# vsislab/Controllable_XGating

Measured on AMD Instinct MI355X. Metric: decoder timesteps/sec (train fwd+bwd) at batch 128, MSRVTT 26x1536+1024, higher is better.
Workload: dtype f32; 1 GPU; configs[1]: 1xMI355X batch 128 per GPU teacher-forced XE train, 26 frames x (1536+1024), hidden 512, att 1536, emb 468, vocab 20000, seq_len 20 (T=21), fp32; global_batch=128, per_gpu_batch=128, parallelism=dp1, gemm_precision=fp32, zero_grad=fused into the update, launch=eager kernel launches

## Files before the change

### controllable_xgating_amd/_native.py

```python
from __future__ import annotations

import ctypes as C
import os

_HERE = os.path.dirname(os.path.abspath(__file__))
LIB_PATH = os.environ.get("XG_LIBRARY") or os.path.join(_HERE, "lib", "libxgate_hip.so")
LIB_DIAG_PATH = os.path.join(_HERE, "lib", "libxgate_hip_diag.so")

XG_VERSION = 206
XG_ROLLOUT_GREEDY, XG_ROLLOUT_SAMPLE, XG_ROLLOUT_REPLAY = 0, 1, 2


class XgDims(C.Structure):
    _fields_ = [(n, C.c_int32) for n in ("B", "K", "R", "A", "E", "V", "C", "H", "F1", "F2", "T")]


class XgBnState(C.Structure):
    _fields_ = [(n, C.c_void_p) for n in ("rgb_mean", "rgb_var", "opfl_mean", "opfl_var")]


class XgBatch(C.Structure):
    _fields_ = [(n, C.c_void_p) for n in ("feats_rgb", "feats_opfl", "feat_mask", "pos_feats", "seq", "seq_mask")]


# ... 79 lines not shown
        "xg_nll_bwd": [vp, vp, vp, vp, i32, i32, i32, i32, vp, f32, vp, vp],
        "xg_clip_adam": [vp, i64, vp, vp, vp, vp, f32, f32, f32, f32, f32, i32, f32],
        "xg_clip_adam_zero": [vp, i64, vp, vp, vp, vp, f32, f32, f32, f32, f32, i32, f32],
        "xg_workspace_init": [vp, vp, C.c_size_t],
        "xg_adam_tick": [vp, vp, f32, f32],
        "xg_clip_adam_dev": [vp, i64, vp, vp, vp, vp, vp, f32, f32, f32, f32, f32, i32],
        "xg_pack_weights": [vp, PD, PP, vp, C.c_size_t, i32, i32],
        "xg_pack_weights_part": [vp, PD, PP, vp, C.c_size_t, i32, i32, i32],
        "xg_reward_fwd": [vp, vp, i32, vp, i32, vp, i32, i32, vp, i32, i32, vp],
        "xg_reward_bwd": [vp, vp, i32, vp, i32, i32, vp, i32, i32, vp, vp, vp, i32],
    }
    missing = [n for n in sigs if not hasattr(L, n)]
    if missing:
        raise XgError("%s (xg_version %d) lacks %s: rebuild it with `python __graft_entry__.py --force`"
                      % (LIB_PATH, L.xg_version(), ", ".join(missing)))
    for name, args in sigs.items():
        fn = getattr(L, name)
        fn.restype = C.c_int
        fn.argtypes = args
    L.xg_abi_check.restype = C.c_int
    L.xg_abi_check.argtypes = [C.c_int] + [C.c_size_t] * 5
    if L.xg_abi_check(XG_VERSION, C.sizeof(XgDims), C.sizeof(_XgParams), C.sizeof(XgBnState), C.sizeof(XgBatch), C.sizeof(XgRun)):
        raise XgError("%s has ABI version %d / other struct layouts than this binding (XG_VERSION %d): rebuild it with "
                      "`python __graft_entry__.py --force`" % (LIB_PATH, L.xg_version(), XG_VERSION))
    _lib = L
    return L


def check(rc: int, what: str):
    if rc != 0:
# ... 14 lines not shown
```

### controllable_xgating_amd/csrc/xg_gemm.hip

```cpp
#include "xg_common.h"
#include "xg_kernels.h"
#include <cstdio>
#include <cstdlib>
#include <type_traits>

typedef float f32x16 __attribute__((ext_vector_type(16)));
typedef float f32x4 __attribute__((ext_vector_type(4)));

namespace {

constexpr int BKS = 32;
constexpr int LDK = BKS + 4;
constexpr int MCP = 4;

template <int ROWS, bool KC>
struct TileGeom {
    static constexpr int lds_floats = KC ? ROWS * LDK : BKS * (ROWS + MCP);
    static constexpr int nvec = ROWS * BKS / 4 / 256;
};

template <int ROWS, bool KC, bool VEC>
__device__ __forceinline__ void load_tile(const float* __restrict__ P, int ld, int r0, int k0, int nrows, int K,
                                          f32x4 (&regs)[TileGeom<ROWS, KC>::nvec]) {
    constexpr int NV = TileGeom<ROWS, KC>::nvec;
// ... 124 lines not shown
                    acc[i][j] = __builtin_amdgcn_mfma_f32_32x32x2f32(fa[i][kk], fb[j][kk], acc[i][j], 0, 0, 0);
    }
}

struct GemmArgs {
    const float* A; const float* B; float* C; const float* bias;
    int M, N, K, lda, ldb, ldc, relu, accumulate;
    int splitk;
    int fast;
    int gm;
    int bg;
    float* csum[3];
    int alone;
};

template <int BM>
__device__ __forceinline__ void csum_flush(const f32x4& cs, f32x4* red4, int m0, int M, float* const (&out)[3]) {
    constexpr int RG = BM / 4;
    const int t = threadIdx.x;
    if (t < RG) {
        f32x4 v = cs;
#pragma unroll
        for (int j = 1; j < 256 / RG; ++j) v += red4[t + j * RG];
#pragma unroll
        for (int q = 0; q < 4; ++q) {
            const int row = m0 + 4 * t + q;
            if (row < M) {
#pragma unroll
                for (int o = 0; o < 3; ++o) if (out[o]) unsafeAtomicAdd(out[o] + row, v[q]);
            }
        }
    }
}

template <int BM, int BN, bool AKC, bool BKC, bool VEC>
__global__ void __launch_bounds__(256) gemm_kernel(GemmArgs g) {
    constexpr int WM = BM / 2, WN = BN / 2;
    constexpr int MT = WM / 32, NT = WN / 32;
    constexpr int A_FL = TileGeom<BM, AKC>::lds_floats;
    constexpr int B_FL = TileGeom<BN, BKC>::lds_floats;
    extern __shared__ __attribute__((aligned(16))) float smem[];
    constexpr int STAGE = A_FL + B_FL;

    const int ntm = (g.M + BM - 1) / BM, ntn = (g.N + BN - 1) / BN;
    const int nwg = ntm * ntn * g.splitk;
    int bid = blockIdx.x;
    {
        const int q = nwg / 8, r = nwg % 8, xcd = bid % 8, idx = bid / 8;
        bid = (xcd < r ? xcd * (q + 1) : r * (q + 1) + (xcd - r) * q) + idx;
    }
    const int ks = bid % g.splitk;
    bid /= g.splitk;
    int tm, tn;
    {
        const int per = g.gm * ntn, grp = bid / per, in = bid - grp * per;
        const int first = grp * g.gm, gsz = min(ntm - first, g.gm);
        tn = in / gsz;
        tm = first + (in - tn * gsz);
    }
    const int m0 = tm * BM, n0 = tn * BN;

    const int lane = threadIdx.x & 63, wave = threadIdx.x >> 6;
    const int wm = wave >> 1, wn = wave & 1;
    const int half = lane >> 5, l31 = lane & 31;

    f32x16 acc[MT][NT];
#pragma unroll
    for (int i = 0; i < MT; ++i)
#pragma unroll
        for (int j = 0; j < NT; ++j)
#pragma unroll
            for (int r = 0; r < 16; ++r) acc[i][j][r] = 0.f;

// ... 1 lines not shown
    f32x4 ra[NVA], rb[NVB];
    const int nslab_all = (g.K + BKS - 1) / BKS;
    const int s_begin = (int)(((long)ks * nslab_all) / g.splitk), s_end = (int)(((long)(ks + 1) * nslab_all) / g.splitk);
    const int nslab = s_end;
    uint32_t offA[NVA], offB[NVB];
    const bool fast = VEC && g.fast;
    if (fast) {
        tile_offsets<BM, AKC>(g.lda, m0, g.M, offA);
        tile_offsets<BN, BKC>(g.ldb, n0, g.N, offB);
    }
    const size_t stepA = (AKC ? (size_t)BKS : (size_t)BKS * g.lda) * sizeof(float);
    const size_t stepB = (BKC ? (size_t)BKS : (size_t)BKS * g.ldb) * sizeof(float);
    const int nfull = g.K / BKS;
    load_tile<BM, AKC, VEC>(g.A, g.lda, m0, s_begin * BKS, g.M, g.K, ra);
    load_tile<BN, BKC, VEC>(g.B, g.ldb, n0, s_begin * BKS, g.N, g.K, rb);
    const bool do_cs = !AKC && VEC && g.csum[0] != nullptr && tn == 0;
    f32x4 cs = {0.f, 0.f, 0.f, 0.f};
    if (do_cs) {
#pragma unroll
        for (int i = 0; i < NVA; ++i) cs += ra[i];
    }
    store_tile<BM, AKC>(smem, ra);
    store_tile<BN, BKC>(smem + A_FL, rb);
    __syncthreads();

    for (int s = s_begin; s < nslab; ++s) {
        const int cur = (s - s_begin) & 1;
        if (s + 1 < nslab) {
            if (fast && s + 1 < nfull) {
                load_fast<NVA>(reinterpret_cast<const char*>(g.A) + (size_t)(s + 1) * stepA, offA, ra);
                load_fast<NVB>(reinterpret_cast<const char*>(g.B) + (size_t)(s + 1) * stepB, offB, rb);
// ... 30 lines not shown
            if (col >= g.N) continue;
            const float bv = (g.bias && ks == 0) ? g.bias[col] : 0.f;
#pragma unroll
            for (int r = 0; r < 16; ++r) {
                const int row = m0 + wm * WM + i * 32 + (r & 3) + 8 * (r >> 2) + 4 * half;
                if (row < g.M) {
                    float* dst = g.C + (size_t)row * g.ldc + col;
                    float v = acc[i][j][r] + bv;
                    if (g.splitk > 1) { unsafeAtomicAdd(dst, v); continue; }
                    if (g.accumulate) v += *dst;
                    if (g.relu) v = fmaxf(v, 0.f);
                    *dst = v;
                }
            }
        }
}

template <int ROWS, int BK, bool KC>
struct TileW {
    static constexpr int ld = KC ? BK + 4 : ROWS + MCP;
    static constexpr int lds_floats = KC ? ROWS * (BK + 4) : BK * (ROWS + MCP);
    static constexpr int nvec = ROWS * BK / 4 / 256;
    static_assert(ROWS * BK % 1024 == 0, "tile must divide over 256 threads");
};
template <int ROWS, int BK, bool KC>
__device__ __forceinline__ void w1_offsets(int ld, int r0, int nrows, uint32_t (&off)[TileW<ROWS, BK, KC>::nvec]) {
    const int t = threadIdx.x;
#pragma unroll
    for (int i = 0; i < TileW<ROWS, BK, KC>::nvec; ++i) {
        const int f = t + 256 * i;
// ... 523 lines not shown
        XG_TRY(xg_lds_optin(optin, reinterpret_cast<const void*>(&gemm_kernel<BM, BN, AKC, BKC, VEC>), (int)lds));
    }
    hipLaunchKernelGGL((gemm_kernel<BM, BN, AKC, BKC, VEC>), dim3(ntm * ntn * g.splitk), dim3(256), lds, st, g);
    XG_CHECK_LAUNCH();
    return XG_OK;
}

struct TdArgs {
    const float* A; const float* B; float* C;
    int M, N, K, lda, ldb, ldc, accumulate;
    int ntm, ntn, ksplit, nrounds;
    float* csum[3];
};
constexpr int TD_LDW = 68;

template <int D>
__global__ void __launch_bounds__(256) gemm_td_kernel(TdArgs g) {
    extern __shared__ __attribute__((aligned(16))) float smem[];
    const int lane = threadIdx.x & 63, wave = __builtin_amdgcn_readfirstlane(threadIdx.x >> 6);
    const int a16 = lane & 15, kq = lane >> 4;
    const int G = gridDim.x;
    const int xq = G >> 3, xr = G & 7, xcd = blockIdx.x & 7, idx = blockIdx.x >> 3;
    const int pos = (xcd < xr ? xcd * (xq + 1) : xr * (xq + 1) + (xcd - xr) * xq) + idx;
    const int nitems = g.ntm * g.ntn * g.ksplit;
    const bool want_cs = g.csum[0] != nullptr;
    const size_t stepA = (size_t)16 * g.lda * sizeof(float), stepB = (size_t)16 * g.ldb * sizeof(float);
    float* red = smem + 4 * 64 * TD_LDW;
    for (int item = pos; item < nitems; item += G) {
        const int part = item % g.ksplit, tile = item / g.ksplit;
        const int tn = tile % g.ntn, tm = tile / g.ntn;
        const int m0 = tm * 64, n0 = tn * 64;
        const int i0 = (int)(((long)part * g.nrounds) / g.ksplit), i1 = (int)(((long)(part + 1) * g.nrounds) / g.ksplit);
        const bool cs_on = want_cs && tn == 0;
        const uint32_t offA = (uint32_t)(((size_t)kq * g.lda + min(m0 + 4 * a16, g.M - 4)) * sizeof(float));
        const uint32_t offB = (uint32_t)(((size_t)kq * g.ldb + min(n0 + 4 * a16, g.N - 4)) * sizeof(float));
        const char* pa = reinterpret_cast<const char*>(g.A) + (size_t)4 * wave * g.lda * sizeof(float);
        const char* pb = reinterpret_cast<const char*>(g.B) + (size_t)4 * wave * g.ldb * sizeof(float);
        f32x4 acc[4][4];
#pragma unroll
        for (int i = 0; i < 4; ++i)
#pragma unroll
            for (int j = 0; j < 4; ++j) acc[i][j] = f32x4{0.f, 0.f, 0.f, 0.f};
        f32x4 cs = {0.f, 0.f, 0.f, 0.f};
        f32x4 ra[D], rb[D];
        const char* qa = pa + (size_t)i0 * stepA;
        const char* qb = pb + (size_t)i0 * stepB;
#pragma unroll
        for (int u = 0; u < D; ++u) {
            ra[u] = *reinterpret_cast<const f32x4*>(qa + u * stepA + offA);
            rb[u] = *reinterpret_cast<const f32x4*>(qb + u * stepB + offB);
        }
        qa += D * stepA; qb += D * stepB;
// ... 40 lines not shown
                v += __shfl_xor(v, 32);
                if (kq == 0) red[wave * 64 + 4 * a16 + q] = v;
            }
        }
        __syncthreads();
        {
            const bool atom = g.ksplit > 1;
#pragma unroll
            for (int u = 0; u < 4; ++u) {
                const int q = lane + 64 * u;
                const int row = 16 * wave + (q >> 4), col = (q & 15) << 2;
                f32x4 v = *reinterpret_cast<const f32x4*>(smem + row * TD_LDW + col);
#pragma unroll
                for (int w2 = 1; w2 < 4; ++w2) v += *reinterpret_cast<const f32x4*>(smem + (w2 * 64 + row) * TD_LDW + col);
                const int gr = m0 + row, gc = n0 + col;
                if (gr < g.M && gc < g.N) {
                    float* dst = g.C + (size_t)gr * g.ldc + gc;
                    if (atom) {
#pragma unroll
                        for (int e = 0; e < 4; ++e) unsafeAtomicAdd(dst + e, v[e]);
                    } else if (g.accumulate) {
                        *reinterpret_cast<f32x4*>(dst) = *reinterpret_cast<const f32x4*>(dst) + v;
                    } else {
                        *reinterpret_cast<f32x4*>(dst) = v;
                    }
                }
            }
            if (cs_on && threadIdx.x < 64) {
                const int m = m0 + (int)threadIdx.x;
                if (m < g.M) {
                    const float v = (red[threadIdx.x] + red[64 + threadIdx.x]) + (red[128 + threadIdx.x] + red[192 + threadIdx.x]);
#pragma unroll
                    for (int o = 0; o < 3; ++o) if (g.csum[o]) unsafeAtomicAdd(g.csum[o] + m, v);
                }
            }
        }
        __syncthreads();
    }
}

int launch_td(hipStream_t st, const GemmArgs& a) {
    static const int off = xg_diag_env("XG_GEMM_NO_TD") ? 1 : 0;
    if (off || !a.fast || a.relu || a.bias || a.M % 4 || a.N % 4 || a.K % 16 || a.ldc % 4 || ((uintptr_t)a.C % 16) != 0) return 1;
    if (a.M < 64 || a.N < 64 || a.K < 16 * 16) return 1;
    TdArgs g{a.A, a.B, a.C, a.M, a.N, a.K, a.lda, a.ldb, a.ldc, a.accumulate, 0, 0, 1, a.K / 16, {a.csum[0], a.csum[1], a.csum[2]}};
    g.ntm = xg_cdiv(a.M, 64); g.ntn = xg_cdiv(a.N, 64);
    const long tiles = (long)g.ntm * g.ntn;
    if (tiles < 32) return 1;
    static const int td_all = xg_diag_env("XG_TD_ALL") ? atoi(xg_diag_env("XG_TD_ALL")) : 0;
    if (!td_all && !a.bg && !a.alone && tiles < 1024) return 1;
    static const int ks_env = xg_diag_env("XG_TD_KS") ? atoi(xg_diag_env("XG_TD_KS")) : 0;
    int ks = 1;
    if (tiles < 192) { ks = (int)(256 / tiles); if (ks > g.nrounds / 16) ks = g.nrounds / 16; if (ks < 1) ks = 1; }
    if (ks_env > 0) ks = ks_env;
    if (ks > g.nrounds / 8) ks = g.nrounds / 8;
    g.ksplit = ks;
    if (ks > 1 && !a.accumulate) {
        if (a.ldc == a.N) { if (hipMemsetAsync(a.C, 0, sizeof(float) * (size_t)a.M * a.N, st) != hipSuccess) return XG_EHIP; }
        else if (hipMemset2DAsync(a.C, sizeof(float) * a.ldc, 0, sizeof(float) * a.N, a.M, st) != hipSuccess) return XG_EHIP;
    }
    static const int bg_off = xg_diag_env("XG_GEMM_NO_BG") ? 1 : 0;
    const bool bg = a.bg && !bg_off;
    const long items = tiles * ks;
    const int GMAX = bg ? 256 : 512;
    const long rounds = xg_cdiv64(items, GMAX);
    const int G = (int)xg_cdiv64(items, rounds);
    size_t lds = (4 * 64 * TD_LDW + 256) * sizeof(float);
    if (bg && lds < 82 * 1024) lds = 82 * 1024;
    static const int depth_all = xg_diag_env("XG_TD_DEPTH") ? atoi(xg_diag_env("XG_TD_DEPTH")) : 8;
    const int depth_env = depth_all;
    if (depth_env == 4) {
        static std::atomic<unsigned> optin4{0};
        XG_TRY(xg_lds_optin(optin4, reinterpret_cast<const void*>(&gemm_td_kernel<4>), 84 * 1024));
        hipLaunchKernelGGL((gemm_td_kernel<4>), dim3(G), dim3(256), lds, st, g);
    } else if (depth_env == 12 && g.nrounds / ks >= 12) {
        static std::atomic<unsigned> optin12{0};
        XG_TRY(xg_lds_optin(optin12, reinterpret_cast<const void*>(&gemm_td_kernel<12>), 84 * 1024));
        hipLaunchKernelGGL((gemm_td_kernel<12>), dim3(G), dim3(256), lds, st, g);
    } else {
        static std::atomic<unsigned> optin{0};
        XG_TRY(xg_lds_optin(optin, reinterpret_cast<const void*>(&gemm_td_kernel<8>), 84 * 1024));
        hipLaunchKernelGGL((gemm_td_kernel<8>), dim3(G), dim3(256), lds, st, g);
    }
    XG_CHECK_LAUNCH();
    return XG_OK;
}
// ... 81 lines not shown
        }
    }
    if (vec && !force) {
        const int rc1 = dispatch_w1<AKC, BKC>(st, g);
        if (rc1 != 1) return rc1;
    }
    if (vec && !force) {
        const int rc = launch_pk<128, 128, AKC, BKC>(st, g, 40);
        if (rc != 1) return rc;
    }
    g.gm = xgk_group_rows(g.K / g.splitk);
    if (big) return vec ? launch<128, 128, AKC, BKC, true>(st, g) : launch<128, 128, AKC, BKC, false>(st, g);
    return vec ? launch<64, 64, AKC, BKC, true>(st, g) : launch<64, 64, AKC, BKC, false>(st, g);
}

}

int xgk_gemm(hipStream_t st, int mode, bool transA, bool transB, int M, int N, int K, const float* A, int lda,
             const float* B, int ldb, float* C, int ldc, const float* bias, bool relu, bool accumulate) {
    return xgk_gemm_cs(st, mode, transA, transB, M, N, K, A, lda, B, ldb, C, ldc, bias, relu, accumulate, nullptr, nullptr, nullptr);
}

int xgk_gemm_cs(hipStream_t st, int mode, bool transA, bool transB, int M, int N, int K, const float* A, int lda,
                const float* B, int ldb, float* C, int ldc, const float* bias, bool relu, bool accumulate, float* cs1, float* cs2,
                float* cs3) {
    if (M <= 0 || N <= 0) return XG_OK;
    if (K < 0 || !A || !B || !C) return XG_EINVAL;
    const bool want_cs = cs1 != nullptr;
    if (want_cs && !transA) return XG_EINVAL;
    const int bg = (mode & XGK_GEMM_BG) ? 1 : 0, alone = (mode & XGK_GEMM_ALONE) ? 1 : 0;
// ... 31 lines not shown
        return xgk_gemm_bf16x(st, 1 | (mode & XGK_GEMM_BG), transA, transB, M, N, K, A, A16, lda, B, B16, ldb, C, ldc, bias, relu, accumulate, cs1, cs2, cs3);
    }
    return xgk_gemm_cs(st, mode, transA, transB, M, N, K, A, lda, B, ldb, C, ldc, bias, relu, accumulate, cs1, cs2, cs3);
}

extern "C" int xg_gemm_mode(void* stream, int mode, int transA, int transB, int M, int N, int K, const float* A, int lda,
                            const float* B, int ldb, float* C, int ldc, const float* bias, int relu, int accumulate) {
    if (mode != 0 && mode != 1 && mode != 3) return XG_EINVAL;
    if (mode == 0 || M <= 0 || N <= 0)
        return xgk_gemm((hipStream_t)stream, 0, transA != 0, transB != 0, M, N, K, A, lda, B, ldb, C, ldc, bias, relu != 0, accumulate != 0);
    if (K < 0 || !A || !B || !C) return XG_EINVAL;
    return xgk_gemm_bf16((hipStream_t)stream, mode, transA != 0, transB != 0, M, N, K, A, lda, B, ldb, C, ldc, bias,
                         relu != 0, accumulate != 0);
}

extern "C" int xg_gemm(void* stream, int transA, int transB, int M, int N, int K, const float* A, int lda,
                       const float* B, int ldb, float* C, int ldc, const float* bias, int relu, int accumulate) {
    return xgk_gemm((hipStream_t)stream, 0, transA != 0, transB != 0, M, N, K, A, lda, B, ldb, C, ldc, bias,
                    relu != 0, accumulate != 0);
}
```

### controllable_xgating_amd/csrc/xg_kernels.h

```cpp
#pragma once
#include "xg_common.h"
#include "xg_select.h"
#include "xg_beam_core.h"
#include <cstddef>

static inline int xgk_group_rows(int k_depth) {
    const int g = 4096 / (k_depth > 0 ? k_depth : 1);
    return g < 1 ? 1 : (g > 8 ? 8 : g);
}
enum { XGK_GEMM_BG = 0x100,
       XGK_GEMM_ALONE = 0x200 };
int xgk_gemm(hipStream_t st, int mode, bool transA, bool transB, int M, int N, int K, const float* A, int lda,
             const float* B, int ldb, float* C, int ldc, const float* bias, bool relu, bool accumulate);
int xgk_gemm_cs(hipStream_t st, int mode, bool transA, bool transB, int M, int N, int K, const float* A, int lda,
                const float* B, int ldb, float* C, int ldc, const float* bias, bool relu, bool accumulate, float* cs1, float* cs2,
                float* cs3);
int xgk_gemm_x(hipStream_t st, int mode, bool transA, bool transB, int M, int N, int K, const float* A, const unsigned short* A16,
               int lda, const float* B, const unsigned short* B16, int ldb, float* C, int ldc, const float* bias, bool relu,
               bool accumulate, float* cs1 = nullptr, float* cs2 = nullptr, float* cs3 = nullptr);
int xgk_gemm_bf16(hipStream_t st, int planes, bool transA, bool transB, int M, int N, int K, const float* A, int lda,
                  const float* B, int ldb, float* C, int ldc, const float* bias, bool relu, bool accumulate, float* cs1 = nullptr,
                  float* cs2 = nullptr, float* cs3 = nullptr);
int xgk_gemm_bf16x(hipStream_t st, int planes, bool transA, bool transB, int M, int N, int K, const float* A, const unsigned short* A16,
                   int lda, const float* B, const unsigned short* B16, int ldb, float* C, int ldc, const float* bias, bool relu,
                   bool accumulate, float* cs1 = nullptr, float* cs2 = nullptr, float* cs3 = nullptr);
bool xgk_gemm_g16_ok(bool transA, bool transB, int M, int N, int K, const unsigned short* A16, int lda, const unsigned short* B16, int ldb);
int xgk_gemm_g16(hipStream_t st, bool transA, bool transB, int M, int N, int K, const unsigned short* A16, int lda,
                 const unsigned short* B16, int ldb, float* C, int ldc, const float* bias, bool relu, bool accumulate, int splitk,
                 float* cs1, float* cs2, float* cs3);
int xgk_cvt_bf16(hipStream_t st, const float* src, unsigned short* dst, size_t n);
static inline int xgk_linear(hipStream_t st, int mode, int M, int N, int K, const float* X, int ldx, const float* W,
                             const float* bias, float* Y, int ldy, bool relu = false, bool acc = false) {
    return xgk_gemm(st, mode, false, true, M, N, K, X, ldx, W, K, Y, ldy, bias, relu, acc);
}
// ... 237 lines not shown
```

### controllable_xgating_amd/csrc/xg_model.hip

```cpp
#include "xg_common.h"
#include <cstring>
#include "xg_kernels.h"
#include "../../include/xgate_beam.h"
#include "../../include/xgate_control.h"
#include "../../include/xgate_beam_control.h"

#include <new>
#include <cstdlib>

namespace {

constexpr int XG_NEV = 64, XG_NRING = 56;
struct XgAux { uint32_t magic; int device; hipStream_t s = nullptr, s2 = nullptr; hipEvent_t ev[XG_NEV]; };
constexpr uint32_t XG_AUX_MAGIC = 0x58474158u;
XgAux* aux_of(const XgRun* run) {
    static const bool disabled = xg_diag_env("XG_NO_OVERLAP") != nullptr;
    if (disabled || !run || !run->aux) return nullptr;
    XgAux* a = static_cast<XgAux*>(run->aux);
    int dev = -1;
    if (a->magic != XG_AUX_MAGIC || hipGetDevice(&dev) != hipSuccess || dev != a->device) return nullptr;
    return a;
}

struct Streams {
// ... 144 lines not shown
    return (!event || hipEventRecord(static_cast<hipEvent_t>(event), st) == hipSuccess) ? XG_OK : XG_EHIP;
}

inline int gemm_nn(hipStream_t st, int mode, int M, int N, int Kc, const float* dY, int lddy, const float* W, int ldw,
                   float* dX, int lddx, bool acc) {
    return xgk_gemm(st, mode, false, false, M, N, Kc, dY, lddy, W, ldw, dX, lddx, nullptr, false, acc);
}
inline int gemm_tn(hipStream_t st, int mode, int Mrows, int N, int K, const float* dY, int lddy, const float* X, int ldx,
                   float* dW, int lddw) {
    return xgk_gemm(st, mode, true, false, N, K, Mrows, dY, lddy, X, ldx, dW, lddw, nullptr, false, true);
}

inline int gemm_tn_cs(hipStream_t st, int mode, int Mrows, int N, int K, const float* dY, int lddy, const float* X, int ldx,
                      float* dW, int lddw, float* b1, float* b2 = nullptr, float* b3 = nullptr) {
    return xgk_gemm_cs(st, mode, true, false, N, K, Mrows, dY, lddy, X, ldx, dW, lddw, nullptr, false, true, b1, b2, b3);
}

inline const unsigned short* m16(const Ws& w, const float* p) {
    return (w.gm == 1 && w.sh16 && p >= w.base_f && p < w.end_f) ? w.sh16 + (p - w.base_f) : nullptr;
}
inline int cvt16(hipStream_t st, const Ws& w, const float* p, size_t n) {
    if (w.gm != 1 || n == 0) return XG_OK;
    if (!w.sh16) return XG_OK;
    const unsigned short* dst = m16(w, p);
    if (!dst) return XG_EINVAL;
    return xgk_cvt_bf16(st, p, const_cast<unsigned short*>(dst), n);
}
inline const unsigned short* w16(const Ws& w, int which) {
    return (w.gm == 1 && w.packed && w.pk.dtype == 1) ? w.pk.w16[which] : nullptr;
}
// ... 225 lines not shown
                sk.job[m].seg[0] = seg_nn(w, mo[m].pkb, w.dS[m] + (size_t)i * 4 * R, K * 4 * R, mo[m].whh, R, 4 * R);
            }
            XG_TRY(xgk_skinny(st, sk, sk_mode(w)));
        }
    }
    for (int m = 0; m < 2; ++m) XG_TRY(cvt16(st, w, w.dS[m], (size_t)N * 4 * R));
    const int gm_tail = w.gm | XGK_GEMM_ALONE;
    XG_TRY(ss.fork2());
    for (int m = 0; m < 2; ++m) {
        const EncMod &e = mo[m], &ge = gr[m];
        if (m == 0) XG_TRY(ss.fork());
        ZERO(sx, w.Hprev[m], (size_t)N * R);
        if (K > 1)
            XG_TRY(xgk_copy2d(sx, w.Hprev[m] + R, K * R, w.Hs[m], K * R, B, (K - 1) * R, false));
        XG_TRY(cvt16(sx, w, w.Hprev[m], (size_t)N * R));
        XG_TRY(tn16(sx, gm_tail, N, 4 * R, R, w.dS[m], m16(w, w.dS[m]), 4 * R, w.Hprev[m], m16(w, w.Hprev[m]), R, ge.whh, R, ge.bih, ge.bhh));
        XG_TRY(tn16(sx, gm_tail, N, 4 * R, R, w.dS[m], m16(w, w.dS[m]), 4 * R, w.X[m], m16(w, w.X[m]), R, ge.wih, R));
        hipStream_t sm = (m == 1 && ss.overlap()) ? ss.aux2 : st;
        XG_TRY(nn16(sm, w.gm, N, R, 4 * R, w.dS[m], m16(w, w.dS[m]), 4 * R, e.wih, w16(w, e.w16_wih), R, w.dX[m], R, false));
        if (!w.zeroed) { ZERO(sm, w.bn_s1[m], R); ZERO(sm, w.bn_s2[m], R); }
        XG_TRY(xgk_bn_bwd_reduce(sm, w.dX[m], w.X[m], w.Z[m], w.bn_mean[m], w.bn_var[m], x.feat_mask, N, R, run.bn_eps,
                                 xg_make_drop(&run, e.site, 0), w.bn_s1[m], w.bn_s2[m]));
        XG_TRY(xgk_bn_bwd_apply(sm, w.dX[m], w.Z[m], w.bn_mean[m], w.bn_var[m], e.bn_g, w.bn_s1[m], w.bn_s2[m], N, R,
                                run.bn_eps, run.train != 0, ge.bn_b, ge.bn_g));
        XG_TRY(gemm_tn_cs(sm, gm_tail, N, R, e.F, w.dX[m], R, e.feats, e.F, ge.emb_w, e.F, ge.emb_b));
    }
    return ss.chain2_into_aux();
}

int init_hidden(hipStream_t st, const XgDims& d, const XgParams& p, const float* V, const float* feat_mask, Ws& w,
                float* h1, float* c1, float* h2, float* c2) {
    const int B = d.B, R = d.R;
// ... 408 lines not shown
        j.ksplit_cap = 4; j.low_prio = 1;
        XG_TRY(xgk_skinny(s1, sk, sk_mode(w)));
        cur1 ^= 1;
        return XG_OK;
    };
    const int wgm = w.gm;
    auto wgrads_chain2 = [=, &w](hipStream_t sq, int t0, int t1) -> int {
        const int rows = (t1 - t0) * B;
        if (rows <= 0) return XG_OK;
        const size_t r0 = (size_t)t0 * B;
        const float* ds2 = w.DS2 + r0 * 4 * R;
        const float* dp = w.DP + r0 * A;
        const float *h1n = w.H1 + BR + r0 * R, *h1 = w.H1 + r0 * R, *h2 = w.H2 + r0 * R, *af = w.AF + r0 * R;
        XG_TRY(cvt16(sq, w, ds2, (size_t)rows * 4 * R)); XG_TRY(cvt16(sq, w, dp, (size_t)rows * A));
        XG_TRY(cvt16(sq, w, h1, (size_t)(rows + B) * R)); XG_TRY(cvt16(sq, w, h2, (size_t)rows * R)); XG_TRY(cvt16(sq, w, af, (size_t)rows * R));
        XG_TRY(tn16(sq, wgm, rows, 4 * R, R, ds2, m16(w, ds2), 4 * R, h1n, m16(w, h1n), R, g.l2_i2h_w, R, g.l2_i2h_b, g.l2_a2h_b, g.l2_h2h_b));
        XG_TRY(tn16(sq, wgm, rows, 4 * R, R, ds2, m16(w, ds2), 4 * R, af, m16(w, af), R, g.l2_a2h_w, R));
        XG_TRY(tn16(sq, wgm, rows, 4 * R, R, ds2, m16(w, ds2), 4 * R, h2, m16(w, h2), R, g.l2_h2h_w, R));
        XG_TRY(tn16(sq, wgm, rows, A, R, dp, m16(w, dp), A, h1, m16(w, h1), R, g.h2a_w, 2 * R, g.h2a_b));
        XG_TRY(tn16(sq, wgm, rows, A, R, dp, m16(w, dp), A, h2, m16(w, h2), R, g.h2a_w + R, 2 * R));
        return XG_OK;
    };
    auto wgrads_chain1 = [=, &w](hipStream_t sq, int t0, int t1) -> int {
        const int rows = (t1 - t0) * B;
        if (rows <= 0) return XG_OK;
        const size_t r0 = (size_t)t0 * B;
        const float* ds1 = w.DS1 + r0 * 4 * R;
        const float *h1 = w.H1 + r0 * R, *posg = w.POSG + r0 * R;
        XG_TRY(cvt16(sq, w, ds1, (size_t)rows * 4 * R)); XG_TRY(cvt16(sq, w, h1, (size_t)rows * R)); XG_TRY(cvt16(sq, w, posg, (size_t)rows * R));
        XG_TRY(tn16(sq, wgm, rows, 4 * R, R, ds1, m16(w, ds1), 4 * R, h1, m16(w, h1), R, g.l1_h2h_w, R, g.l1_i2h_b, g.l1_a2h_b, g.l1_h2h_b));
        XG_TRY(tn16(sq, wgm, rows, 4 * R, E, ds1, m16(w, ds1), 4 * R, w.Xe + r0 * E, nullptr, E, g.l1_i2h_w, E));
        XG_TRY(tn16(sq, wgm, rows, 4 * R, R, ds1, m16(w, ds1), 4 * R, posg, m16(w, posg), R, g.l1_a2h_w, R));
        XG_TRY(nn16(sq, wgm, rows, R, 4 * R, ds1, m16(w, ds1), 4 * R, p.l1_a2h_w, w16(w, W16_L1_A2H), R, w.DPOSG + r0 * R, R, false));
        XG_TRY(nn16(sq, wgm, rows, E, 4 * R, ds1, m16(w, ds1), 4 * R, p.l1_i2h_w, w16(w, W16_L1_I2H), E, w.DXe + r0 * E, E, false));
        return XG_OK;
    };
    const int wg_chunks = (ss.overlap() && T >= 8 && w.gm == 0) ? 2 : 1;
    int wg_hi = T, wg_mark = -1;
    int c1_next = T - 1;
    for (int t = T - 1; t >= 0; --t) {
        if (t == ss.dh_split_step - (fuse ? 0 : 1)) XG_TRY(ss.wait_mark(ss.dh_mark));
        float* dh2p = w.dst[cur ^ 1][2];
        float* ds2 = w.DS2 + (size_t)t * B * 4 * R;
        float* dp = w.DP + (size_t)t * B * A;
        float* daf = w.DAF + t * BR;
        if (!fuse || t == T - 1) XG_TRY(xgk_lstm_bwd(st, cell_bwd(2, t, cur, w.DH2OUT + t * BR)));
        {
// ... 956 lines not shown
```

### include/xgate.h

```cpp
#ifndef XGATE_H
#define XGATE_H

#include <stddef.h>
#include <stdint.h>

#ifdef __cplusplus
extern "C" {
#endif

#define XG_VERSION 206

enum {
    XG_OK = 0,
    XG_EINVAL = -1,
    XG_EARCH = -2,
    XG_EHIP = -3,
    XG_EWORKSPACE = -4
};

typedef struct XgDims {
    int32_t B, K, R, A, E, V, C, H, F1, F2, T;
} XgDims;

typedef struct XgParams {
// ... 48 lines not shown
int xg_abi_check(int version, size_t sz_dims, size_t sz_params, size_t sz_bn, size_t sz_batch, size_t sz_run);
const char *xg_strerror(int code);
int xg_param_count(void);
const char *xg_param_name(int index);
int xg_param_numel(const XgDims *d, int index, int64_t *numel);
size_t xg_workspace_bytes(const XgDims *d);
size_t xg_workspace_bytes_mode(const XgDims *d, int gemm_mode);
int xg_workspace_init(void *stream, void *ws, size_t ws_bytes);

int xg_gemm(void *stream, int transA, int transB, int M, int N, int K,
            const float *A, int lda, const float *B, int ldb, float *C, int ldc,
            const float *bias, int relu, int accumulate);
int xg_gemm_mode(void *stream, int mode, int transA, int transB, int M, int N, int K,
                 const float *A, int lda, const float *B, int ldb, float *C, int ldc,
                 const float *bias, int relu, int accumulate);

int xg_gemm_bf16_operands(void *stream, int transA, int transB, int M, int N, int K, const float *A, const void *A16, int lda,
                          const float *B, const void *B16, int ldb, float *C, int ldc, const float *bias, int relu, int accumulate);
int xg_cvt_bf16(void *stream, const float *src, void *dst , int64_t n);

int xg_encoder_fwd(void *stream, const XgDims *d, const XgParams *p, const XgBnState *bn,
                   const XgBatch *x, const XgRun *run, void *ws, size_t ws_bytes,
                   float *V );
int xg_encoder_bwd(void *stream, const XgDims *d, const XgParams *p, const XgParams *g,
                   const XgBatch *x, const XgRun *run, void *ws, size_t ws_bytes,
                   const float *dV);

int xg_init_hidden(void *stream, const XgDims *d, const XgParams *p, const float *V,
                   const float *feat_mask, void *ws, size_t ws_bytes, float *state);

// ... 91 lines not shown
```

Baseline: 513,500 decoder timesteps/s.

## Batch weight-gradient GEMMs sharing one dY operand into a single concatenated launch

Adds a concatenated-N GEMM path (gemm_cat_kernel and a TD variant) in which several weight-gradient GEMMs that share the same dY (A) operand are tiled together in one launch, each tile picking its B/C block via a small block table. This cuts kernel-launch count and lets small per-weight GEMMs fill the GPU together instead of running serially. The path is wired into the encoder LSTM backward and decoder weight-gradient chains behind a site mask, and the default mask enables only the encoder site (bit 8). The risk is extra per-tile indexing and different split-k and tiling choices for the merged shape.

```diff
diff --git a/controllable_xgating_amd/_native.py b/controllable_xgating_amd/_native.py
--- a/controllable_xgating_amd/_native.py
+++ b/controllable_xgating_amd/_native.py
@@ -117,6 +117,9 @@
     if missing:
         raise XgError("%s (xg_version %d) lacks %s: rebuild it with `python __graft_entry__.py --force`"
                       % (LIB_PATH, L.xg_version(), ", ".join(missing)))
+    if hasattr(L, "xg_gemm_cat"):
+        sigs["xg_gemm_cat"] = [vp, i32, i32, vp, i32, i32, C.POINTER(vp), C.POINTER(i32), C.POINTER(i32), C.POINTER(vp),
+                               C.POINTER(i32), i32, vp, vp, vp]
     for name, args in sigs.items():
         fn = getattr(L, name)
         fn.restype = C.c_int
diff --git a/controllable_xgating_amd/csrc/xg_gemm.hip b/controllable_xgating_amd/csrc/xg_gemm.hip
--- a/controllable_xgating_amd/csrc/xg_gemm.hip
+++ b/controllable_xgating_amd/csrc/xg_gemm.hip
@@ -162,6 +162,19 @@
     int alone;
 };
 
+struct CatBlocks {
+    int nblk;
+    int t0[XGK_CAT_MAX + 1];
+    const float* B[XGK_CAT_MAX]; float* C[XGK_CAT_MAX];
+    int ldb[XGK_CAT_MAX], ldc[XGK_CAT_MAX], n[XGK_CAT_MAX];
+};
+__device__ __forceinline__ int cat_block_of(const CatBlocks& cb, int tn) {
+    int j = 0;
+#pragma unroll
+    for (int q = 1; q < XGK_CAT_MAX; ++q) if (q < cb.nblk && tn >= cb.t0[q]) j = q;
+    return j;
+}
+
 template <int BM>
 __device__ __forceinline__ void csum_flush(const f32x4& cs, f32x4* red4, int m0, int M, float* const (&out)[3]) {
     constexpr int RG = BM / 4;
@@ -181,8 +194,8 @@
     }
 }
 
-template <int BM, int BN, bool AKC, bool BKC, bool VEC>
-__global__ void __launch_bounds__(256) gemm_kernel(GemmArgs g) {
+template <int BM, int BN, bool AKC, bool BKC, bool VEC, bool CAT>
+__device__ __forceinline__ void gemm_body(GemmArgs g, const CatBlocks* cb) {
     constexpr int WM = BM / 2, WN = BN / 2;
     constexpr int MT = WM / 32, NT = WN / 32;
     constexpr int A_FL = TileGeom<BM, AKC>::lds_floats;
@@ -190,7 +203,7 @@
     extern __shared__ __attribute__((aligned(16))) float smem[];
     constexpr int STAGE = A_FL + B_FL;
 
-    const int ntm = (g.M + BM - 1) / BM, ntn = (g.N + BN - 1) / BN;
+    const int ntm = (g.M + BM - 1) / BM, ntn = CAT ? cb->t0[XGK_CAT_MAX] : (g.N + BN - 1) / BN;
     const int nwg = ntm * ntn * g.splitk;
     int bid = blockIdx.x;
     {
@@ -205,6 +218,13 @@
         const int first = grp * g.gm, gsz = min(ntm - first, g.gm);
         tn = in / gsz;
         tm = first + (in - tn * gsz);
+    }
+    const bool col0 = tn == 0;
+    if constexpr (CAT) {
+        const int j = cat_block_of(*cb, tn);
+        tn -= cb->t0[j];
+        g.B = cb->B[j]; g.ldb = cb->ldb[j]; g.N = cb->n[j];
+        g.C = cb->C[j]; g.ldc = cb->ldc[j];
     }
     const int m0 = tm * BM, n0 = tn * BN;
 
@@ -236,7 +256,7 @@
     const int nfull = g.K / BKS;
     load_tile<BM, AKC, VEC>(g.A, g.lda, m0, s_begin * BKS, g.M, g.K, ra);
     load_tile<BN, BKC, VEC>(g.B, g.ldb, n0, s_begin * BKS, g.N, g.K, rb);
-    const bool do_cs = !AKC && VEC && g.csum[0] != nullptr && tn == 0;
+    const bool do_cs = !AKC && VEC && g.csum[0] != nullptr && col0;
     f32x4 cs = {0.f, 0.f, 0.f, 0.f};
     if (do_cs) {
 #pragma unroll
@@ -297,6 +317,15 @@
                 }
             }
         }
+}
+
+template <int BM, int BN, bool AKC, bool BKC, bool VEC>
+__global__ void __launch_bounds__(256) gemm_kernel(GemmArgs g) {
+    gemm_body<BM, BN, AKC, BKC, VEC, false>(g, nullptr);
+}
+template <int BM, int BN>
+__global__ void __launch_bounds__(256) gemm_cat_kernel(GemmArgs g, CatBlocks cb) {
+    gemm_body<BM, BN, false, false, true, true>(g, &cb);
 }
 
 template <int ROWS, int BK, bool KC>
@@ -850,8 +879,8 @@
 };
 constexpr int TD_LDW = 68;
 
-template <int D>
-__global__ void __launch_bounds__(256) gemm_td_kernel(TdArgs g) {
+template <int D, bool CAT>
+__device__ __forceinline__ void gemm_td_body(const TdArgs& g, const CatBlocks* cb) {
     extern __shared__ __attribute__((aligned(16))) float smem[];
     const int lane = threadIdx.x & 63, wave = __builtin_amdgcn_readfirstlane(threadIdx.x >> 6);
     const int a16 = lane & 15, kq = lane >> 4;
@@ -860,18 +889,28 @@
     const int pos = (xcd < xr ? xcd * (xq + 1) : xr * (xq + 1) + (xcd - xr) * xq) + idx;
     const int nitems = g.ntm * g.ntn * g.ksplit;
     const bool want_cs = g.csum[0] != nullptr;
-    const size_t stepA = (size_t)16 * g.lda * sizeof(float), stepB = (size_t)16 * g.ldb * sizeof(float);
+    const size_t stepA = (size_t)16 * g.lda * sizeof(float);
     float* red = smem + 4 * 64 * TD_LDW;
     for (int item = pos; item < nitems; item += G) {
         const int part = item % g.ksplit, tile = item / g.ksplit;
-        const int tn = tile % g.ntn, tm = tile / g.ntn;
+        int tn = tile % g.ntn;
+        const int tm = tile / g.ntn;
+        const bool cs_on = want_cs && tn == 0;
+        const float* Bp = g.B; float* Cp = g.C;
+        int ldb = g.ldb, ldc = g.ldc, N = g.N;
+        if constexpr (CAT) {
+            const int j = cat_block_of(*cb, tn);
+            tn -= cb->t0[j];
+            Bp = cb->B[j]; ldb = cb->ldb[j]; N = cb->n[j];
+            Cp = cb->C[j]; ldc = cb->ldc[j];
+        }
+        const size_t stepB = (size_t)16 * ldb * sizeof(float);
         const int m0 = tm * 64, n0 = tn * 64;
         const int i0 = (int)(((long)part * g.nrounds) / g.ksplit), i1 = (int)(((long)(part + 1) * g.nrounds) / g.ksplit);
-        const bool cs_on = want_cs && tn == 0;
         const uint32_t offA = (uint32_t)(((size_t)kq * g.lda + min(m0 + 4 * a16, g.M - 4)) * sizeof(float));
-        const uint32_t offB = (uint32_t)(((size_t)kq * g.ldb + min(n0 + 4 * a16, g.N - 4)) * sizeof(float));
+        const uint32_t offB = (uint32_t)(((size_t)kq * ldb + min(n0 + 4 * a16, N - 4)) * sizeof(float));
         const char* pa = reinterpret_cast<const char*>(g.A) + (size_t)4 * wave * g.lda * sizeof(float);
-        const char* pb = reinterpret_cast<const char*>(g.B) + (size_t)4 * wave * g.ldb * sizeof(float);
+        const char* pb = reinterpret_cast<const char*>(Bp) + (size_t)4 * wave * ldb * sizeof(float);
         f32x4 acc[4][4];
 #pragma unroll
         for (int i = 0; i < 4; ++i)
@@ -942,8 +981,8 @@
 #pragma unroll
                 for (int w2 = 1; w2 < 4; ++w2) v += *reinterpret_cast<const f32x4*>(smem + (w2 * 64 + row) * TD_LDW + col);
                 const int gr = m0 + row, gc = n0 + col;
-                if (gr < g.M && gc < g.N) {
-                    float* dst = g.C + (size_t)gr * g.ldc + gc;
+                if (gr < g.M && gc < N) {
+                    float* dst = Cp + (size_t)gr * ldc + gc;
                     if (atom) {
 #pragma unroll
                         for (int e = 0; e < 4; ++e) unsafeAtomicAdd(dst + e, v[e]);
@@ -966,13 +1005,42 @@
         __syncthreads();
     }
 }
-
-int launch_td(hipStream_t st, const GemmArgs& a) {
+template <int D>
+__global__ void __launch_bounds__(256) gemm_td_kernel(TdArgs g) {
+    gemm_td_body<D, false>(g, nullptr);
+}
+__global__ void __launch_bounds__(256) gemm_td_cat_kernel(TdArgs g, CatBlocks cb) {
+    gemm_td_body<8, true>(g, &cb);
+}
+
+int zero_outputs(hipStream_t st, const GemmArgs& a, const CatBlocks* cb) {
+    const int nb = cb ? cb->nblk : 1;
+    for (int j = 0; j < nb; ++j) {
+        float* C = cb ? cb->C[j] : a.C;
+        const int ldc = cb ? cb->ldc[j] : a.ldc, N = cb ? cb->n[j] : a.N;
+        if (ldc == N) { if (hipMemsetAsync(C, 0, sizeof(float) * (size_t)a.M * N, st) != hipSuccess) return XG_EHIP; }
+        else if (hipMemset2DAsync(C, sizeof(float) * ldc, 0, sizeof(float) * N, a.M, st) != hipSuccess) return XG_EHIP;
+    }
+    return XG_OK;
+}
+
+int launch_td(hipStream_t st, const GemmArgs& a, const CatBlocks* cb = nullptr) {
     static const int off = xg_diag_env("XG_GEMM_NO_TD") ? 1 : 0;
-    if (off || !a.fast || a.relu || a.bias || a.M % 4 || a.N % 4 || a.K % 16 || a.ldc % 4 || ((uintptr_t)a.C % 16) != 0) return 1;
+    if (off || !a.fast || a.relu || a.bias || a.M % 4 || a.K % 16) return 1;
+    for (int j = 0; j < (cb ? cb->nblk : 1); ++j) {
+        const int N = cb ? cb->n[j] : a.N, ldc = cb ? cb->ldc[j] : a.ldc;
+        if (N % 4 || N < 4 || ldc % 4 || ((uintptr_t)(cb ? cb->C[j] : a.C) % 16) != 0) return 1;
+    }
     if (a.M < 64 || a.N < 64 || a.K < 16 * 16) return 1;
     TdArgs g{a.A, a.B, a.C, a.M, a.N, a.K, a.lda, a.ldb, a.ldc, a.accumulate, 0, 0, 1, a.K / 16, {a.csum[0], a.csum[1], a.csum[2]}};
     g.ntm = xg_cdiv(a.M, 64); g.ntn = xg_cdiv(a.N, 64);
+    CatBlocks c{};
+    if (cb) {
+        c = *cb;
+        int t = 0;
+        for (int j = 0; j <= XGK_CAT_MAX; ++j) { c.t0[j] = t; if (j < c.nblk) t += xg_cdiv(c.n[j], 64); }
+        g.ntn = t;
+    }
     const long tiles = (long)g.ntm * g.ntn;
     if (tiles < 32) return 1;
     static const int td_all = xg_diag_env("XG_TD_ALL") ? atoi(xg_diag_env("XG_TD_ALL")) : 0;
@@ -983,10 +1051,7 @@
     if (ks_env > 0) ks = ks_env;
     if (ks > g.nrounds / 8) ks = g.nrounds / 8;
     g.ksplit = ks;
-    if (ks > 1 && !a.accumulate) {
-        if (a.ldc == a.N) { if (hipMemsetAsync(a.C, 0, sizeof(float) * (size_t)a.M * a.N, st) != hipSuccess) return XG_EHIP; }
-        else if (hipMemset2DAsync(a.C, sizeof(float) * a.ldc, 0, sizeof(float) * a.N, a.M, st) != hipSuccess) return XG_EHIP;
-    }
+    if (ks > 1 && !a.accumulate) XG_TRY(zero_outputs(st, a, cb));
     static const int bg_off = xg_diag_env("XG_GEMM_NO_BG") ? 1 : 0;
     const bool bg = a.bg && !bg_off;
     const long items = tiles * ks;
@@ -997,7 +1062,11 @@
     if (bg && lds < 82 * 1024) lds = 82 * 1024;
     static const int depth_all = xg_diag_env("XG_TD_DEPTH") ? atoi(xg_diag_env("XG_TD_DEPTH")) : 8;
     const int depth_env = depth_all;
-    if (depth_env == 4) {
+    if (cb) {
+        static std::atomic<unsigned> optinc{0};
+        XG_TRY(xg_lds_optin(optinc, reinterpret_cast<const void*>(&gemm_td_cat_kernel), 84 * 1024));
+        hipLaunchKernelGGL(gemm_td_cat_kernel, dim3(G), dim3(256), lds, st, g, c);
+    } else if (depth_env == 4) {
         static std::atomic<unsigned> optin4{0};
         XG_TRY(xg_lds_optin(optin4, reinterpret_cast<const void*>(&gemm_td_kernel<4>), 84 * 1024));
         hipLaunchKernelGGL((gemm_td_kernel<4>), dim3(G), dim3(256), lds, st, g);
@@ -1109,6 +1178,87 @@
     return vec ? launch<64, 64, AKC, BKC, true>(st, g) : launch<64, 64, AKC, BKC, false>(st, g);
 }
 
+template <int BM, int BN>
+int launch_cat(hipStream_t st, const GemmArgs& g, CatBlocks cb) {
+    int t = 0;
+    for (int j = 0; j <= XGK_CAT_MAX; ++j) { cb.t0[j] = t; if (j < cb.nblk) t += xg_cdiv(cb.n[j], BN); }
+    const int ntm = xg_cdiv(g.M, BM);
+    if (g.splitk > 1 && !g.accumulate) XG_TRY(zero_outputs(st, g, &cb));
+    const size_t lds = 2 * (TileGeom<BM, false>::lds_floats + TileGeom<BN, false>::lds_floats) * sizeof(float);
+    if (lds > 65536) {
+        static std::atomic<unsigned> optin{0};
+        XG_TRY(xg_lds_optin(optin, reinterpret_cast<const void*>(&gemm_cat_kernel<BM, BN>), (int)lds));
+    }
+    hipLaunchKernelGGL((gemm_cat_kernel<BM, BN>), dim3(ntm * t * g.splitk), dim3(256), lds, st, g, cb);
+    XG_CHECK_LAUNCH();
+    return XG_OK;
+}
+
+int dispatch_cat(hipStream_t st, GemmArgs g, const CatBlocks& cb) {
+    long c128 = 0, c64 = 0;
+    for (int j = 0; j < cb.nblk; ++j) { c128 += xg_cdiv(cb.n[j], 128); c64 += xg_cdiv(cb.n[j], 64); }
+    const long t128 = xg_cdiv(g.M, 128) * c128, t64 = xg_cdiv(g.M, 64) * c64;
+    const int nslab = xg_cdiv(g.K, BKS);
+    bool big = t128 >= 1024;
+    g.splitk = 1;
+    if (!big) {
+        long sk = 768 / (t64 > 0 ? t64 : 1);
+        if (sk > nslab / 16) sk = nslab / 16;
+        if (sk >= 2) g.splitk = (int)sk;
+    }
+    static const char* force_all = xg_diag_env("XG_GEMM_FORCE");
+    static const char* force_cat = xg_diag_env("XG_CAT_FORCE");
+    const char* force = force_all ? force_all : force_cat;
+    if (force) {
+        int t = 0, sk = 1;
+        if (sscanf(force, "%d,%d", &t, &sk) == 2) { big = t == 128; g.splitk = sk < 1 ? 1 : sk; }
+    }
+    if (g.splitk > nslab) g.splitk = nslab > 0 ? nslab : 1;
+    if (!force) {
+        g.gm = xgk_group_rows(g.K);
+        const int rct = launch_td(st, g, &cb);
+        if (rct != 1) return rct;
+    }
+    g.gm = xgk_group_rows(g.K / g.splitk);
+    return big ? launch_cat<128, 128>(st, g, cb) : launch_cat<64, 64>(st, g, cb);
+}
+
+}
+
+int xgk_gemm_tn_cat(hipStream_t st, int mode, int M, int K, const float* A, int lda, int nblk, const XgkCatBlock* blk,
+                    bool accumulate, float* cs1, float* cs2, float* cs3) {
+    if (nblk < 1 || nblk > XGK_CAT_MAX || !blk) return XG_EINVAL;
+    if (M <= 0) return XG_OK;
+    if (K < 0 || !A) return XG_EINVAL;
+    const int base_mode = mode & ~(XGK_GEMM_BG | XGK_GEMM_ALONE);
+    bool vec = base_mode == 0 && K > 0 && ((uintptr_t)A % 16 == 0) && lda % 4 == 0 && M % 4 == 0 && M >= 4;
+    bool fast = (size_t)K * lda * 4 < (1u << 31);
+    CatBlocks cb{};
+    long ntot = 0;
+    for (int j = 0; j < nblk; ++j) {
+        const XgkCatBlock& b = blk[j];
+        if (b.n <= 0) { vec = false; continue; }
+        if (!b.B || !b.C) return XG_EINVAL;
+        vec = vec && ((uintptr_t)b.B % 16 == 0) && b.ldb % 4 == 0 && b.n % 4 == 0;
+        fast = fast && (size_t)K * b.ldb * 4 < (1u << 31);
+        cb.B[j] = b.B; cb.C[j] = b.C; cb.ldb[j] = b.ldb; cb.ldc[j] = b.ldc; cb.n[j] = b.n;
+        ntot += b.n;
+    }
+    if (!vec || ntot > (1 << 30)) {
+        for (int j = 0; j < nblk; ++j) {
+            const XgkCatBlock& b = blk[j];
+            if (b.n <= 0) continue;
+            const bool first = cs1 != nullptr;
+            XG_TRY(xgk_gemm_x(st, mode, true, false, M, b.n, K, A, nullptr, lda, b.B, nullptr, b.ldb, b.C, b.ldc, nullptr, false, accumulate,
+                              first ? cs1 : nullptr, first ? cs2 : nullptr, first ? cs3 : nullptr));
+            cs1 = nullptr;
+        }
+        return XG_OK;
+    }
+    cb.nblk = nblk;
+    GemmArgs g{A, cb.B[0], cb.C[0], nullptr, M, (int)ntot, K, lda, cb.ldb[0], cb.ldc[0], 0, accumulate ? 1 : 0, 1, fast ? 1 : 0, 1, 0,
+               {cs1, cs2, cs3}, (mode & XGK_GEMM_ALONE) ? 1 : 0};
+    return dispatch_cat(st, g, cb);
 }
 
 int xgk_gemm(hipStream_t st, int mode, bool transA, bool transB, int M, int N, int K, const float* A, int lda,
@@ -1170,6 +1320,15 @@
                          relu != 0, accumulate != 0);
 }
 
+extern "C" int xg_gemm_cat(void* stream, int M, int K, const float* A, int lda, int nblk, const float* const* B, const int* ldb,
+                           const int* n, float* const* C, const int* ldc, int accumulate, float* cs1, float* cs2, float* cs3) {
+    if (nblk < 1 || nblk > XGK_CAT_MAX || !B || !ldb || !n || !C || !ldc) return XG_EINVAL;
+    if (!cs1 && (cs2 || cs3)) return XG_EINVAL;
+    XgkCatBlock blk[XGK_CAT_MAX];
+    for (int j = 0; j < nblk; ++j) blk[j] = XgkCatBlock{B[j], ldb[j], n[j], C[j], ldc[j]};
+    return xgk_gemm_tn_cat((hipStream_t)stream, 0, M, K, A, lda, nblk, blk, accumulate != 0, cs1, cs2, cs3);
+}
+
 extern "C" int xg_gemm(void* stream, int transA, int transB, int M, int N, int K, const float* A, int lda,
                        const float* B, int ldb, float* C, int ldc, const float* bias, int relu, int accumulate) {
     return xgk_gemm((hipStream_t)stream, 0, transA != 0, transB != 0, M, N, K, A, lda, B, ldb, C, ldc, bias,
diff --git a/controllable_xgating_amd/csrc/xg_kernels.h b/controllable_xgating_amd/csrc/xg_kernels.h
--- a/controllable_xgating_amd/csrc/xg_kernels.h
+++ b/controllable_xgating_amd/csrc/xg_kernels.h
@@ -18,6 +18,10 @@
 int xgk_gemm_x(hipStream_t st, int mode, bool transA, bool transB, int M, int N, int K, const float* A, const unsigned short* A16,
                int lda, const float* B, const unsigned short* B16, int ldb, float* C, int ldc, const float* bias, bool relu,
                bool accumulate, float* cs1 = nullptr, float* cs2 = nullptr, float* cs3 = nullptr);
+struct XgkCatBlock { const float* B; int ldb; int n; float* C; int ldc; };
+constexpr int XGK_CAT_MAX = 3;
+int xgk_gemm_tn_cat(hipStream_t st, int mode, int M, int K, const float* A, int lda, int nblk, const XgkCatBlock* blk,
+                    bool accumulate, float* cs1 = nullptr, float* cs2 = nullptr, float* cs3 = nullptr);
 int xgk_gemm_bf16(hipStream_t st, int planes, bool transA, bool transB, int M, int N, int K, const float* A, int lda,
                   const float* B, int ldb, float* C, int ldc, const float* bias, bool relu, bool accumulate, float* cs1 = nullptr,
                   float* cs2 = nullptr, float* cs3 = nullptr);
diff --git a/controllable_xgating_amd/csrc/xg_model.hip b/controllable_xgating_amd/csrc/xg_model.hip
--- a/controllable_xgating_amd/csrc/xg_model.hip
+++ b/controllable_xgating_amd/csrc/xg_model.hip
@@ -182,6 +182,14 @@
 inline int gemm_tn_cs(hipStream_t st, int mode, int Mrows, int N, int K, const float* dY, int lddy, const float* X, int ldx,
                       float* dW, int lddw, float* b1, float* b2 = nullptr, float* b3 = nullptr) {
     return xgk_gemm_cs(st, mode, true, false, N, K, Mrows, dY, lddy, X, ldx, dW, lddw, nullptr, false, true, b1, b2, b3);
+}
+
+#ifndef XG_CAT_SITES_DEFAULT
+#define XG_CAT_SITES_DEFAULT 8
+#endif
+inline bool cat_site(int gm, int bit) {
+    static const int mask = xg_diag_env("XG_CAT_SITES") ? atoi(xg_diag_env("XG_CAT_SITES")) : XG_CAT_SITES_DEFAULT;
+    return gm == 0 && (mask & bit) != 0;
 }
 
 inline const unsigned short* m16(const Ws& w, const float* p) {
@@ -437,8 +445,13 @@
         if (K > 1)
             XG_TRY(xgk_copy2d(sx, w.Hprev[m] + R, K * R, w.Hs[m], K * R, B, (K - 1) * R, false));
         XG_TRY(cvt16(sx, w, w.Hprev[m], (size_t)N * R));
-        XG_TRY(tn16(sx, gm_tail, N, 4 * R, R, w.dS[m], m16(w, w.dS[m]), 4 * R, w.Hprev[m], m16(w, w.Hprev[m]), R, ge.whh, R, ge.bih, ge.bhh));
-        XG_TRY(tn16(sx, gm_tail, N, 4 * R, R, w.dS[m], m16(w, w.dS[m]), 4 * R, w.X[m], m16(w, w.X[m]), R, ge.wih, R));
+        if (cat_site(w.gm, 8)) {
+            const XgkCatBlock b[2] = {{w.Hprev[m], R, R, ge.whh, R}, {w.X[m], R, R, ge.wih, R}};
+            XG_TRY(xgk_gemm_tn_cat(sx, gm_tail, 4 * R, N, w.dS[m], 4 * R, 2, b, true, ge.bih, ge.bhh));
+        } else {
+            XG_TRY(tn16(sx, gm_tail, N, 4 * R, R, w.dS[m], m16(w, w.dS[m]), 4 * R, w.Hprev[m], m16(w, w.Hprev[m]), R, ge.whh, R, ge.bih, ge.bhh));
+            XG_TRY(tn16(sx, gm_tail, N, 4 * R, R, w.dS[m], m16(w, w.dS[m]), 4 * R, w.X[m], m16(w, w.X[m]), R, ge.wih, R));
+        }
         hipStream_t sm = (m == 1 && ss.overlap()) ? ss.aux2 : st;
         XG_TRY(nn16(sm, w.gm, N, R, 4 * R, w.dS[m], m16(w, w.dS[m]), 4 * R, e.wih, w16(w, e.w16_wih), R, w.dX[m], R, false));
         if (!w.zeroed) { ZERO(sm, w.bn_s1[m], R); ZERO(sm, w.bn_s2[m], R); }
@@ -877,11 +890,21 @@
         const float *h1n = w.H1 + BR + r0 * R, *h1 = w.H1 + r0 * R, *h2 = w.H2 + r0 * R, *af = w.AF + r0 * R;
         XG_TRY(cvt16(sq, w, ds2, (size_t)rows * 4 * R)); XG_TRY(cvt16(sq, w, dp, (size_t)rows * A));
         XG_TRY(cvt16(sq, w, h1, (size_t)(rows + B) * R)); XG_TRY(cvt16(sq, w, h2, (size_t)rows * R)); XG_TRY(cvt16(sq, w, af, (size_t)rows * R));
-        XG_TRY(tn16(sq, wgm, rows, 4 * R, R, ds2, m16(w, ds2), 4 * R, h1n, m16(w, h1n), R, g.l2_i2h_w, R, g.l2_i2h_b, g.l2_a2h_b, g.l2_h2h_b));
-        XG_TRY(tn16(sq, wgm, rows, 4 * R, R, ds2, m16(w, ds2), 4 * R, af, m16(w, af), R, g.l2_a2h_w, R));
-        XG_TRY(tn16(sq, wgm, rows, 4 * R, R, ds2, m16(w, ds2), 4 * R, h2, m16(w, h2), R, g.l2_h2h_w, R));
-        XG_TRY(tn16(sq, wgm, rows, A, R, dp, m16(w, dp), A, h1, m16(w, h1), R, g.h2a_w, 2 * R, g.h2a_b));
-        XG_TRY(tn16(sq, wgm, rows, A, R, dp, m16(w, dp), A, h2, m16(w, h2), R, g.h2a_w + R, 2 * R));
+        if (cat_site(wgm, 1)) {
+            const XgkCatBlock b[3] = {{h1n, R, R, g.l2_i2h_w, R}, {af, R, R, g.l2_a2h_w, R}, {h2, R, R, g.l2_h2h_w, R}};
+            XG_TRY(xgk_gemm_tn_cat(sq, wgm, 4 * R, rows, ds2, 4 * R, 3, b, true, g.l2_i2h_b, g.l2_a2h_b, g.l2_h2h_b));
+        } else {
+            XG_TRY(tn16(sq, wgm, rows, 4 * R, R, ds2, m16(w, ds2), 4 * R, h1n, m16(w, h1n), R, g.l2_i2h_w, R, g.l2_i2h_b, g.l2_a2h_b, g.l2_h2h_b));
+            XG_TRY(tn16(sq, wgm, rows, 4 * R, R, ds2, m16(w, ds2), 4 * R, af, m16(w, af), R, g.l2_a2h_w, R));
+            XG_TRY(tn16(sq, wgm, rows, 4 * R, R, ds2, m16(w, ds2), 4 * R, h2, m16(w, h2), R, g.l2_h2h_w, R));
+        }
+        if (cat_site(wgm, 2)) {
+            const XgkCatBlock b[2] = {{h1, R, R, g.h2a_w, 2 * R}, {h2, R, R, g.h2a_w + R, 2 * R}};
+            XG_TRY(xgk_gemm_tn_cat(sq, wgm, A, rows, dp, A, 2, b, true, g.h2a_b));
+        } else {
+            XG_TRY(tn16(sq, wgm, rows, A, R, dp, m16(w, dp), A, h1, m16(w, h1), R, g.h2a_w, 2 * R, g.h2a_b));
+            XG_TRY(tn16(sq, wgm, rows, A, R, dp, m16(w, dp), A, h2, m16(w, h2), R, g.h2a_w + R, 2 * R));
+        }
         return XG_OK;
     };
     auto wgrads_chain1 = [=, &w](hipStream_t sq, int t0, int t1) -> int {
@@ -891,9 +914,14 @@
         const float* ds1 = w.DS1 + r0 * 4 * R;
         const float *h1 = w.H1 + r0 * R, *posg = w.POSG + r0 * R;
         XG_TRY(cvt16(sq, w, ds1, (size_t)rows * 4 * R)); XG_TRY(cvt16(sq, w, h1, (size_t)rows * R)); XG_TRY(cvt16(sq, w, posg, (size_t)rows * R));
-        XG_TRY(tn16(sq, wgm, rows, 4 * R, R, ds1, m16(w, ds1), 4 * R, h1, m16(w, h1), R, g.l1_h2h_w, R, g.l1_i2h_b, g.l1_a2h_b, g.l1_h2h_b));
-        XG_TRY(tn16(sq, wgm, rows, 4 * R, E, ds1, m16(w, ds1), 4 * R, w.Xe + r0 * E, nullptr, E, g.l1_i2h_w, E));
-        XG_TRY(tn16(sq, wgm, rows, 4 * R, R, ds1, m16(w, ds1), 4 * R, posg, m16(w, posg), R, g.l1_a2h_w, R));
+        if (cat_site(wgm, 4)) {
+            const XgkCatBlock b[3] = {{h1, R, R, g.l1_h2h_w, R}, {w.Xe + r0 * E, E, E, g.l1_i2h_w, E}, {posg, R, R, g.l1_a2h_w, R}};
+            XG_TRY(xgk_gemm_tn_cat(sq, wgm, 4 * R, rows, ds1, 4 * R, 3, b, true, g.l1_i2h_b, g.l1_a2h_b, g.l1_h2h_b));
+        } else {
+            XG_TRY(tn16(sq, wgm, rows, 4 * R, R, ds1, m16(w, ds1), 4 * R, h1, m16(w, h1), R, g.l1_h2h_w, R, g.l1_i2h_b, g.l1_a2h_b, g.l1_h2h_b));
+            XG_TRY(tn16(sq, wgm, rows, 4 * R, E, ds1, m16(w, ds1), 4 * R, w.Xe + r0 * E, nullptr, E, g.l1_i2h_w, E));
+            XG_TRY(tn16(sq, wgm, rows, 4 * R, R, ds1, m16(w, ds1), 4 * R, posg, m16(w, posg), R, g.l1_a2h_w, R));
+        }
         XG_TRY(nn16(sq, wgm, rows, R, 4 * R, ds1, m16(w, ds1), 4 * R, p.l1_a2h_w, w16(w, W16_L1_A2H), R, w.DPOSG + r0 * R, R, false));
         XG_TRY(nn16(sq, wgm, rows, E, 4 * R, ds1, m16(w, ds1), 4 * R, p.l1_i2h_w, w16(w, W16_L1_I2H), E, w.DXe + r0 * E, E, false));
         return XG_OK;
diff --git a/include/xgate.h b/include/xgate.h
--- a/include/xgate.h
+++ b/include/xgate.h
@@ -86,6 +86,10 @@
 int xg_gemm_mode(void *stream, int mode, int transA, int transB, int M, int N, int K,
                  const float *A, int lda, const float *B, int ldb, float *C, int ldc,
                  const float *bias, int relu, int accumulate);
+
+int xg_gemm_cat(void *stream, int M, int K, const float *A, int lda, int nblk,
+                const float *const *B, const int *ldb, const int *n, float *const *C, const int *ldc,
+                int accumulate, float *cs1, float *cs2, float *cs3);
 
 int xg_gemm_bf16_operands(void *stream, int transA, int transB, int M, int N, int K, const float *A, const void *A16, int lda,
                           const float *B, const void *B16, int ldb, float *C, int ldc, const float *bias, int relu, int accumulate);
```

Result: no change. 515,100 decoder timesteps/s, median of 6 (+0.3%).
